# greysun/GraphEmbeddings

Hardware: AMD Instinct MI355X
Metric: scored triples/sec/GPU (d=200) (higher is better)
Workload: dtype f32

## Files before the change

### graphembeddings_amd/csrc/ge_launch.h

```cpp
#pragma once
#include <assert.h>
#include <hip/hip_runtime.h>
#include <stddef.h>
#include <stdint.h>

#include "ge_step_id.h"
#include "ge_sweep_route.h"
#include "ge_trans.h"

namespace ge {

struct TileGeom;
struct ShardOut;

int complex_max_dim();
bool complex_shape_ok(int32_t d, const void* table);
int complex_score_launch(const float* table, int64_t N, int32_t d, const int32_t* triples, int64_t B, float max_norm,
                         int apply_sigmoid, float* out, hipStream_t st, int spectral = 0, float label = 0.f, float l2 = 0.f,
                         const float* table_sumsq = nullptr, int64_t ld = 0);
int complex_hinge_loss_launch(const float* table, int64_t N, int32_t d, const int32_t* pos, const int32_t* neg, int64_t B,
                              float margin, float max_norm, float* loss, float* sig_out, hipStream_t st, int spectral = 0);
int complex_hinge_grad_launch(const float* rows, int64_t N, int32_t d, const int32_t* pos, const int32_t* neg, int64_t B,
                              float margin, float lr, float max_norm, float* loss, int32_t* grad_idx, float* grad_val,
                              hipStream_t st, hipEvent_t ev_start = nullptr, hipEvent_t ev_stop = nullptr,
                              const int32_t* slot_item = nullptr, float* table_rw = nullptr, int spectral = 0,
                              const int32_t* order = nullptr);
int complex_logloss_grad_launch(const float* rows, int64_t N, int32_t d, const int32_t* triples, const float* labels,
                                int64_t M, float lr, float max_norm, float l2, const float* table_sumsq, float* loss,
                                int32_t* grad_idx, float* grad_val, hipStream_t st, const int32_t* negs = nullptr,
                                int64_t B = 0, float row_scale = 1.f, float neg_lr_eff = 0.f, hipEvent_t ev_start = nullptr,
                                hipEvent_t ev_stop = nullptr);
int shard_hinge_grad_launch(float* shard, int32_t d, const float* staged, const int32_t* pos_src, const int32_t* neg_src,
                            const int32_t* slot_item, int32_t R, int64_t B, float margin, float lr, float max_norm,
                            float* loss, int32_t* grad_idx, float* grad_val, float* gsum, int spectral, hipStream_t st,
                            hipEvent_t ev_start, hipEvent_t ev_stop, const int32_t* order, const float* const* peers,
                            int n_peers);
int table_sumsq_launch(const float* table, int64_t n, float* out, hipStream_t st);
int table_scale_launch(float* table, int64_t n, float factor, hipStream_t st);

int hole_max_dim();
int hole_score_launch(const float* table, int64_t N, int32_t d, const int32_t* triples, int64_t B, float max_norm,
                      int apply_sigmoid, float* out, hipStream_t st);
int hole_hinge_loss_launch(const float* table, int64_t N, int32_t d, const int32_t* pos, const int32_t* neg, int64_t B,
                           float margin, float max_norm, float* loss, float* sig_out, hipStream_t st);
int hole_hinge_grad_launch(const float* rows, int64_t N, int32_t d, const int32_t* pos, const int32_t* neg, int64_t B,
                           float margin, float lr, float max_norm, float* loss, int32_t* grad_idx, float* grad_val,
                           hipStream_t st, hipEvent_t ev_start = nullptr, hipEvent_t ev_stop = nullptr);

int hole_spectral_launch(float* table, int64_t N, int32_t d, int inverse, hipStream_t st);

int scatter_add_rows_launch(float* table, int64_t N, int32_t d, const int32_t* idx, const float* val, int64_t R,
                            hipStream_t st, hipEvent_t ev_start = nullptr, hipEvent_t ev_stop = nullptr);
int gather_rows_launch(const float* table, int64_t N, int32_t d, const int32_t* idx, int64_t R, float* out, hipStream_t st);
int corrupt_batch_launch(const int32_t* pos, int64_t B, const TypeSampler& ts, uint64_t step, int32_t* neg, hipStream_t st);
struct SamplerArgs {
  const int32_t* triples; int64_t T; const int64_t* bh_key; const int32_t* bh_ent; const int64_t* bt_key;
  const int32_t* bt_ent; int64_t n_known; const uint32_t* tail_threshold; int32_t n_rel, n_ent;
};
int bernoulli_corrupt_launch(const int32_t* pos, int64_t B, const SamplerArgs& s, int32_t ent_lo, uint64_t seed,
                             uint64_t step, int32_t* neg, hipStream_t st);
int select_rows_launch(const int32_t* valid, int64_t V, int64_t B, uint64_t seed, uint64_t counter, int32_t* out,
                       hipStream_t st);
int mean_pocket_launch(const float* loss, int64_t B, float* mean_out, float* best, int32_t* flag, hipStream_t st);
int copy_if_launch(const float* src, float* dst, int64_t n, const int32_t* flag, hipStream_t st);
bool copy_if_ok(const float* src, const float* dst, int64_t n);
constexpr int kCopyIfChunk = 8192;
// ... 6 lines not shown
int rank_metrics_launch(const int32_t* n_before, const int32_t* n_known_before, const float* true_loss, int64_t M,
                        float* metrics_out, float* best, int32_t* improved, hipStream_t st);

int complex_score_1vK_launch(const float* table, int64_t N, int32_t d, const int32_t* hr, int64_t B, const int32_t* cand,
                             int64_t K, float max_norm, int apply_sigmoid, int cand_is_head, float* out, hipStream_t st);

struct SweepArgs {
  const float* table; int64_t N; int32_t d; const int32_t* hr; int64_t B; const int32_t* true_id; const int32_t* cand;
  int64_t K; float max_norm; int cand_is_head; const int32_t* known_off; const uint16_t* known_rc; int32_t* raw_cnt;
  int32_t* skip_cnt; float* true_loss; float* scores_out; int spec, scores_only, sweep_flags;
};
inline int table_mod16(const SweepArgs& a) { return (int)(reinterpret_cast<uintptr_t>(a.table) % 16); }
struct TopkOut { int32_t k; int32_t* out_id; float* out_loss; void* workspace; size_t workspace_bytes; };
struct SetArgs {
  const int32_t* row_set; const uint32_t* mask; int32_t n_sets;
  int64_t mw;
};

int complex_rank_1vK_launch(const SweepArgs& a, const void* planes_ws, hipStream_t st);

int pipe_sweep_launch(int cw, const SweepArgs& a, hipStream_t st);

int rank_planes_launch(const float* table, int64_t N, int32_t d, const int32_t* cand, int64_t K, float max_norm, int spec,
                       void* planes_ws, hipStream_t st);
int f16_sweep_launch(const SweepArgs& a, const void* planes_ws, hipStream_t st);
int topk_f16_launch(const SweepArgs& a, const TopkOut& t, const void* planes_ws, hipStream_t st);

int64_t candidate_mask_words(int64_t K);
int mask_from_classes_launch(const int32_t* cand_class, int64_t K, const uint32_t* allow, int32_t n_sets, int32_t n_class,
                             uint32_t* mask, hipStream_t st);
int mask_from_cells_launch(const int32_t* cells, int64_t M, int32_t n_sets, int64_t K, uint32_t* mask, hipStream_t st);
int masked_rank_launch(const SweepArgs& a, const SetArgs& sets, const void* planes_ws, hipStream_t st);
int masked_topk_launch(const SweepArgs& a, const TopkOut& t, const SetArgs& sets, const void* planes_ws, hipStream_t st);

int neighbor_max_k();
int neighbor_max_dim();
int64_t neighbor_planes_bytes(int64_t K, int32_t d);
int neighbor_planes_launch(const float* table, int64_t N, int32_t d, const int32_t* cand, int64_t K, void* planes_ws,
                           hipStream_t st);
size_t neighbor_ws_bytes(int64_t B, int64_t K, int32_t k);
int neighbor_dists_launch(const float* table, int64_t N, int32_t d, const int32_t* queries, int64_t B,
                          const int32_t* cand, int64_t K, int metric, const void* planes_ws, float* out, hipStream_t st);
int neighbor_topk_launch(const float* table, int64_t N, int32_t d, const int32_t* queries, int64_t B,
                         const int32_t* cand, int64_t K, int32_t k, int metric, int exclude_self, const void* planes_ws,
                         int32_t* out_id, float* out_dist, void* workspace, size_t workspace_bytes, hipStream_t st);

int known_cells_launch(int pass, const int64_t* key, const int64_t* ent, int64_t M, const int64_t* fixed, const int64_t* rel,
                       int64_t B, const int64_t* pos_of, int64_t n_rows, int64_t n_cand, int32_t* tile_cnt, int32_t* off,
                       uint16_t* rc, hipStream_t st);

size_t sort_scratch_bytes(int64_t n, int64_t n_sub, int64_t P);
unsigned long long* sort_scratch_keys(void* scratch);
int sort_tiles_launch(void* scratch, int64_t n, int64_t n_sub, int64_t P, int64_t n_rows, hipStream_t st,
                      const unsigned* limit, const unsigned long long** sorted);
int items_launch(const unsigned long long* sorted, int64_t n, const TileGeom& G, int direct, int32_t* out, const ShardOut* so,
                 hipStream_t st);
int relation_order_launch(const int32_t* triples, int64_t T, int64_t first_row, int64_t B, int64_t s0, int64_t n, int64_t N,
                          int32_t* out, int64_t stride, int64_t off_order, void* scratch, hipStream_t st);
size_t prep_big_scratch_bytes(int64_t B, int64_t negs, int64_t n);
int prepare_big_launch(const StepSeq& q, int64_t s0, int64_t n, const TypeSampler& ts, int direct, int32_t* out,
                       void* scratch, hipStream_t st, int negs);

int apply_items_launch(float* table, int d, const TileGeom& G, const int32_t* step_rec, const int32_t* gidx,
                       const float* gval, int split, float* out2, hipStream_t st, hipEvent_t ev_start, hipEvent_t ev_stop,
                       int det);
template <class T>
inline T* ws_at(void* base, size_t off) { return reinterpret_cast<T*>(reinterpret_cast<uintptr_t>(base) + off); }
struct HingeWs { int32_t* gidx; float* gval; size_t bytes; };
HingeWs hinge_ws(void* base, int64_t B, int32_t d);
struct LoglossWs { float* sumsq; int32_t* gidx; float* gval; size_t bytes; };
LoglossWs logloss_ws(void* base, int64_t M, int32_t d);
struct StepHyper {
  float lr0, decay_steps, decay_rate, max_norm;
  float lr_at(uint64_t gs) const { return decay_steps > 0.f ? lr0 / (1.0f + decay_rate * ((float)gs / decay_steps)) : lr0; }
};
size_t train_ws_bytes(int64_t B, int32_t d);
int train_steps_run(float* table, int32_t d, const StepSeq& q, int64_t n_steps, const TypeSampler& ts, float margin,
                    const StepHyper& hp, int model, float* loss, int keep_all_losses, int32_t* neg_ws, void* workspace,
                    size_t workspace_bytes, void** ev_pairs, int ev_kernel, void* pipe_handle, hipStream_t st);
size_t train_logloss_ws_bytes(int64_t B, int32_t negs, int32_t d);
int train_logloss_run(float* table, int32_t d, const StepSeq& q, int64_t n_steps, const TypeSampler& ts, int32_t negs,
                      float l2, const StepHyper& hp, float* loss, int keep_all_losses, int32_t* neg_ws, void* workspace,
                      size_t workspace_bytes, void* pipe_handle, hipStream_t st);
size_t train_prepare_bytes(int64_t B, int64_t n_steps);
int train_prepare_run(const StepSeq& q, int64_t n_steps, const TypeSampler& ts, int direct, int32_t* out, hipStream_t st);
void train_prepared_layout(int64_t B, int64_t* out);
int64_t train_chunk_steps(int64_t B, int64_t negs);
int train_adagrad_run(float* table, float* accum, int32_t d, const StepSeq& q, int64_t n_steps, const TypeSampler& ts,
                      float margin, const StepHyper& hp, int model, float* loss, int keep_all_losses, int32_t* neg_ws,
                      void* workspace, size_t workspace_bytes, void* pipe_handle, hipStream_t st);
int pipeline_create(void** out);
int pipeline_reset(void* h);
int pipeline_destroy(void* h);

int adagrad_items_launch(float* table, float* accum, int d, const TileGeom& G, const int32_t* step_rec, const int32_t* gidx,
                         float* gval, float lr, hipStream_t st);
int adagrad_rows_launch(float* table, float* accum, int64_t N, int32_t d, const int32_t* idx, const float* val,
                        const int32_t* perm, int64_t R, float lr, hipStream_t st);

struct SoftmaxWs { float* qp; float* cp; int32_t* qkey; int32_t* ckey; float* lse; float4* part; float* gq; size_t bytes; };
SoftmaxWs softmax_ws(void* base, int64_t B, int64_t K, int32_t d);
size_t softmax_ws_bytes(int64_t B, int64_t K, int32_t d);
int softmax_launch(const float* table, int64_t N, int32_t d, const int32_t* hr, int64_t B, const int32_t* true_id,
                   const int32_t* cand, int64_t K, float max_norm, float scale, float lr, int cand_is_head, float* loss,
                   int32_t* grad_idx, float* grad_val, void* workspace, hipStream_t st);
int softmax_prepare_launch(const float* table, int64_t N, int32_t d, const int32_t* hr, int64_t B, const int32_t* true_id,
                           const int32_t* cand, int64_t K, float max_norm, int cand_is_head, const int32_t* row_set,
                           int32_t n_sets, const SoftmaxWs& w, hipStream_t st);
// ... 174 lines not shown
```

### graphembeddings_amd/csrc/ge_prep.h

```cpp
#pragma once
#include "ge_common.h"

namespace ge {

constexpr int kSlotDirect = -2;
constexpr int kPrepThreads = 1024;
constexpr int kPrepWaves = kPrepThreads / kWave;
constexpr int kItemCap = 16;
constexpr int64_t kSub = 4096;
constexpr int kMaxRadix = 256;
constexpr unsigned long long kInvalidKey = ~0ull;

__host__ __device__ inline int64_t step_row(int64_t first_row, int64_t T, int64_t B, int64_t s) {
  int64_t first = first_row % T;
  if (first + B > T) first = 0;
  const int64_t n0 = (T - first) / B;
  if (s < n0) return first + s * B;
  const int64_t per = T / B;
  return ((s - n0) % per) * B;
}

struct PrepLayout {
  int64_t B, negs, units, n_sub, S, P, off_slot, off_order, off_sub, sub_stride, off_items, off_islots, stride;
  int epu;
// ... 5 lines not shown
  L.epu = negs > 0 ? 3 : 4;
  L.units = negs > 0 ? (1 + negs) * B : B;
  L.n_sub = (L.units + kSub - 1) / kSub;
  const int64_t s = L.units < kSub ? L.units : kSub;
  const int64_t gran = negs > 0 ? 1024 : 256;
  L.S = (s + gran - 1) / gran * gran;
  L.P = L.epu * L.S;
  L.off_slot = 3 * B;
  L.off_order = (negs == 0 && L.n_sub > 1) ? 9 * B : -1;
  L.off_sub = negs > 0 ? (3 * negs * B + 63) / 64 * 64 : ((L.off_order >= 0 ? 10 : 9) * B + 63) / 64 * 64;
  L.off_items = 64;
  L.off_islots = 64 + 2 * L.P;
  L.sub_stride = 64 + 2 * L.P + kItemCap * L.P;
  L.stride = L.off_sub + L.n_sub * L.sub_stride;
  return L;
}

struct TileGeom {
  int P, n_sub;
  int64_t stride;
  int64_t off_slot;
  int64_t off_sub, sub_stride;
  int off_items, off_islots;
};
inline TileGeom geom_of(const PrepLayout& L) {
  return TileGeom{(int)L.P, (int)L.n_sub, L.stride, L.off_slot, L.off_sub, L.sub_stride, (int)L.off_items, (int)L.off_islots};
}
inline TileGeom geom_plain(int P, int n_sub) {
  const int64_t sub = 64 + 2 * (int64_t)P + kItemCap * (int64_t)P;
  return TileGeom{P, n_sub, n_sub * sub, -1, 0, sub, 64, 64 + 2 * P};
}

struct ShardOut {
  int32_t R;
  int64_t B;
  int32_t* pos_src;
  int32_t* neg_src;
  int32_t* req_row;
  const int32_t* tile_heads;
  int32_t peer;
};

struct SortBits { int n_pass, bits; };
inline SortBits sort_bits_for(int64_t N) {
  int nbits = 1;
  while (((int64_t)1 << nbits) <= N) ++nbits;
  SortBits s;
  s.n_pass = (nbits + 7) / 8;
  s.bits = (nbits + s.n_pass - 1) / s.n_pass;
  if (s.bits < 6) s.bits = 6;
  return s;
}

__device__ __forceinline__ int wave_incl_add(int v, int lane) {
#pragma unroll
  for (int o = 1; o < kWave; o <<= 1) { const int t = __shfl_up(v, o, kWave); if (lane >= o) v += t; }
  return v;
}
__device__ __forceinline__ int wave_incl_max(int v, int lane) {
#pragma unroll
  for (int o = 1; o < kWave; o <<= 1) { const int t = __shfl_up(v, o, kWave); if (lane >= o) v = max(v, t); }
  return v;
}

struct StepSource {
  const int32_t* pos; int64_t B; const int32_t* id_to_type; int64_t N; const int64_t* type_offsets;
  int32_t n_types; const int32_t* type_ids; uint64_t seed, step; int32_t padded_size, mode, negs;
};

__device__ __forceinline__ void unit_keys(const StepSource& S, int64_t j, bool batch_heads, int32_t* __restrict__ neg,
                                          unsigned long long (&k)[4]) {
  if (S.negs > 0) {
    const int64_t B = S.B;
    const int64_t i = j < B ? j : (j - B) % B;
    int32_t t3[3] = {S.pos[3 * i], S.pos[3 * i + 1], S.pos[3 * i + 2]};
    if (j >= B) {
      const int64_t kk = (j - B) / B;
      const uint64_t stepk = S.step * (uint64_t)S.negs + (uint64_t)kk;
      const bool heads_k = (S.mode == GE_CORRUPT_BATCH_COIN) ? batch_coin_heads(S.seed, stepk) : false;
      int col;
      const int32_t repl = corrupt_one(t3, i, heads_k, S.id_to_type, S.N, S.type_offsets, S.n_types, S.type_ids, S.seed,
                                       stepk, S.padded_size, S.mode, col);
      t3[col] = repl;
      int32_t* o = neg + 3 * (kk * B + i);
      o[0] = t3[0]; o[1] = t3[1]; o[2] = t3[2];
    }
    const bool bad = t3[0] < 0 || t3[1] < 0 || t3[2] < 0 || t3[0] >= S.N || t3[1] >= S.N || t3[2] >= S.N;
#pragma unroll
    for (int X = 0; X < 3; ++X)
      k[X] = bad ? kInvalidKey : (((unsigned long long)(uint32_t)t3[X] << 32) | (uint32_t)(3 * j + X));
    k[3] = kInvalidKey;
    return;
  }
  const int64_t i = j;
  int32_t p[3] = {S.pos[3 * i], S.pos[3 * i + 1], S.pos[3 * i + 2]};
  int col;
  const int32_t repl = corrupt_one(p, i, batch_heads, S.id_to_type, S.N, S.type_offsets, S.n_types, S.type_ids, S.seed,
                                   S.step, S.padded_size, S.mode, col);
  int32_t n[3] = {p[0], p[1], p[2]};
  n[col] = repl;
  neg[3 * i] = n[0]; neg[3 * i + 1] = n[1]; neg[3 * i + 2] = n[2];
  const bool bad = p[0] < 0 || p[1] < 0 || p[2] < 0 || p[0] >= S.N || p[1] >= S.N || p[2] >= S.N || repl < 0 || repl >= S.N;
#pragma unroll
  for (int X = 0; X < 3; ++X)
    k[X] = bad ? kInvalidKey : (((unsigned long long)(uint32_t)p[X] << 32) | (uint32_t)(6 * i + X));
  k[3] = (bad || repl == p[col]) ? kInvalidKey : (((unsigned long long)(uint32_t)repl << 32) | (uint32_t)(6 * i + 3 + col));
// ... 4 lines not shown
```

### graphembeddings_amd/csrc/ge_prep_big.hip

```cpp
#include "ge_prep.h"
#include "ge_launch.h"
#include <algorithm>

namespace ge {

__global__ __launch_bounds__(kPrepThreads) void prep_big_keys_kernel(
    const int32_t* __restrict__ triples, int64_t T, int64_t first_row, int64_t B, int64_t s0,
    const int32_t* __restrict__ id_to_type, int64_t N, const int64_t* __restrict__ type_offsets,
    int32_t n_types, const int32_t* __restrict__ type_ids, uint64_t seed, uint64_t global_step0,
    int32_t padded_size, int32_t mode, int direct, int negs, int32_t* __restrict__ prep,
    unsigned long long* __restrict__ keys_out) {
  const PrepLayout L = prep_layout(B, negs);
  const int tid = threadIdx.x, sub = blockIdx.y;
  const int64_t s = s0 + blockIdx.x;
  int32_t* rec = prep + (int64_t)blockIdx.x * L.stride;
  int32_t* slot_item = rec + L.off_slot;
  const int64_t i0 = (int64_t)sub * kSub;
  const int S = (int)((L.units - i0) < kSub ? (L.units - i0) : kSub);
  StepSource src{triples + 3 * step_row(first_row, T, B, s), B, id_to_type, N, type_offsets, n_types, type_ids, seed,
                 global_step0 + (uint64_t)s, padded_size, mode, negs};
  const bool batch_heads = (mode == GE_CORRUPT_BATCH_COIN) ? batch_coin_heads(seed, src.step) : false;
  unsigned long long* out = keys_out + ((int64_t)blockIdx.x * L.n_sub + sub) * L.P;
  if (direct)
    for (int i = tid; i < 6 * S; i += kPrepThreads) slot_item[6 * i0 + i] = -1;
  for (int il = tid; il < (int)L.S; il += kPrepThreads) {
    unsigned long long k[4] = {kInvalidKey, kInvalidKey, kInvalidKey, kInvalidKey};
    if (il < S) unit_keys(src, i0 + il, batch_heads, rec, k);
#pragma unroll
    for (int X = 0; X < 4; ++X)
      if (X < L.epu) out[L.epu * il + X] = k[X];
  }
}

__device__ __forceinline__ bool pass_is_identity(const unsigned* limit, int shift) {
  return limit && ((unsigned long long)(*limit) >> (shift - 32)) == 0ull;
}

__global__ __launch_bounds__(kPrepThreads) void prep_big_hist_kernel(
    const unsigned long long* __restrict__ src, int P, int n_sub, int shift, int bits, unsigned* __restrict__ hist,
    const unsigned* __restrict__ limit) {
  __shared__ unsigned cnt[kMaxRadix];
  if (pass_is_identity(limit, shift)) return;
  const int tid = threadIdx.x, tile = blockIdx.y;
  const int radix = 1 << bits;
  const unsigned dmask = (unsigned)radix - 1u;
  if (tid < radix) cnt[tid] = 0;
  __syncthreads();
  const unsigned long long* k = src + ((int64_t)blockIdx.x * n_sub + tile) * P;
  for (int i = tid; i < P; i += kPrepThreads) atomicAdd(&cnt[(unsigned)(k[i] >> shift) & dmask], 1u);
  __syncthreads();
  if (tid < radix) hist[((int64_t)blockIdx.x * radix + tid) * n_sub + tile] = cnt[tid];
}

__global__ __launch_bounds__(kPrepThreads) void prep_big_scatter_kernel(
    const unsigned long long* __restrict__ src, unsigned long long* __restrict__ dst,
    const unsigned* __restrict__ hist, int P, int n_sub, int shift, int bits, const unsigned* __restrict__ limit) {
  __shared__ unsigned whist[kMaxRadix * kPrepWaves];
  __shared__ unsigned gbase[kMaxRadix];
  __shared__ unsigned dstart[kMaxRadix];
  __shared__ unsigned wsum[4], wsum2[4];
  extern __shared__ __attribute__((aligned(16))) unsigned long long lkeys[];
  const int tid = threadIdx.x, lane = tid & (kWave - 1), wave = tid >> 6, tile = blockIdx.y;
  if (pass_is_identity(limit, shift)) {
    const int64_t o = ((int64_t)blockIdx.x * n_sub + tile) * P;
    for (int i = tid; i < P; i += kPrepThreads) dst[o + i] = src[o + i];
    return;
  }
  const int radix = 1 << bits, R = P / kPrepThreads, seg = kWave * R;
  const unsigned dmask = (unsigned)radix - 1u;
  const unsigned* h = hist + (int64_t)blockIdx.x * radix * n_sub;
  unsigned tot = 0, before = 0, mine = 0;
  if (tid < radix)
    for (int q = 0; q < n_sub; ++q) { const unsigned v = h[tid * n_sub + q]; if (q < tile) before += v; if (q == tile) mine = v; tot += v; }
  int incl = 0, incl2 = 0;
  if (tid < kMaxRadix) {
    incl = wave_incl_add((int)tot, lane);
    incl2 = wave_incl_add((int)mine, lane);
    if (lane == kWave - 1) { wsum[wave] = (unsigned)incl; wsum2[wave] = (unsigned)incl2; }
  }
  for (int i = tid; i < radix * kPrepWaves; i += kPrepThreads) whist[i] = 0;
  __syncthreads();
  if (tid < radix) {
    unsigned run = (unsigned)incl - tot, run2 = (unsigned)incl2 - mine;
    for (int w = 0; w < wave; ++w) { run += wsum[w]; run2 += wsum2[w]; }
    gbase[tid] = run + before;
    dstart[tid] = run2;
  }
  const unsigned long long* kin = src + ((int64_t)blockIdx.x * n_sub + tile) * P;
  unsigned long long k[16];
  unsigned off[16];
#pragma unroll
  for (int r = 0; r < 16; ++r)
    if (r < R) k[r] = kin[wave * seg + r * kWave + lane];
#pragma unroll
  for (int r = 0; r < 16; ++r) {
    if (r < R) {
      const unsigned dg = (unsigned)(k[r] >> shift) & dmask;
      unsigned long long peers = ~0ull;
      for (int b = 0; b < bits; ++b) {
        const bool bit = (dg >> b) & 1u;
        const unsigned long long bal = __ballot(bit);
        peers &= bit ? bal : ~bal;
      }
      const unsigned rank = (unsigned)__popcll(peers & ((1ull << lane) - 1ull));
      const unsigned cnt = (unsigned)__popcll(peers);
      unsigned* hp = whist + dg * kPrepWaves + wave;
      const unsigned base = *hp;
      __builtin_amdgcn_wave_barrier();
      if (rank == 0) *hp = base + cnt;
      __builtin_amdgcn_wave_barrier();
      off[r] = base + rank;
    }
  }
  __syncthreads();
  if (tid < radix) {
    unsigned run = 0;
    for (int w = 0; w < kPrepWaves; ++w) { const unsigned c = whist[tid * kPrepWaves + w]; whist[tid * kPrepWaves + w] = run; run += c; }
  }
  __syncthreads();
#pragma unroll
  for (int r = 0; r < 16; ++r) {
    if (r < R) {
      const unsigned dg = (unsigned)(k[r] >> shift) & dmask;
      lkeys[dstart[dg] + whist[dg * kPrepWaves + wave] + off[r]] = k[r];
    }
  }
  __syncthreads();
  unsigned long long* out = dst + (int64_t)blockIdx.x * n_sub * P;
  for (int i = tid; i < P; i += kPrepThreads) {
    const unsigned long long kk = lkeys[i];
    const unsigned dg = (unsigned)(kk >> shift) & dmask;
    out[gbase[dg] + ((unsigned)i - dstart[dg])] = kk;
  }
}

template <bool SHARD>
__global__ __launch_bounds__(kPrepThreads) void prep_big_items_kernel(
    const unsigned long long* __restrict__ sorted, TileGeom G, int direct, int32_t* __restrict__ prep, ShardOut so) {
  extern __shared__ __attribute__((aligned(16))) unsigned long long keys[];
  const int P = G.P, R = P / kPrepThreads, seg = kWave * R, n_sub = G.n_sub;
  int* wtot = reinterpret_cast<int*>(keys + P);
  const int tid = threadIdx.x, lane = tid & (kWave - 1), wave = tid >> 6, tile = blockIdx.y;
  const unsigned long long* g = sorted + (int64_t)blockIdx.x * n_sub * P;
  const int total = n_sub * P, base = tile * P;
  int32_t* rec = prep + (int64_t)blockIdx.x * G.stride;
  int32_t* slot_item = G.off_slot >= 0 ? rec + G.off_slot : nullptr;
  int32_t* subrec = rec + G.off_sub + tile * G.sub_stride;
  int32_t* items = subrec + G.off_items;
  int32_t* islots = subrec + G.off_islots;
  for (int i = tid; i < P; i += kPrepThreads) keys[i] = g[base + i];
  if (tid == 0) {
    int rs = -1;
    if (tile > 0) {
      const unsigned long long k0 = g[base], kp = g[base - 1];
      const uint32_t r0 = (uint32_t)(k0 >> 32);
      if (k0 != kInvalidKey && (uint32_t)(kp >> 32) == r0) {
        int lo = 0, hi = base - 1;
        while (lo < hi) { const int mid = (lo + hi) >> 1; if ((uint32_t)(g[mid] >> 32) < r0) lo = mid + 1; else hi = mid; }
        rs = lo;
      }
    }
    wtot[31] = rs;
    int before = 0;
    if (SHARD)
      for (int t = 0; t < tile; ++t) before += so.tile_heads[(int64_t)blockIdx.x * n_sub + t];
    wtot[30] = before;
  }
  __syncthreads();
  const int rs_in = wtot[31], u_before = wtot[30];
  auto key_at = [&](int i) -> unsigned long long {
    if (i >= 0 && i < P) return keys[i];
    const int gi = base + i;
    return (gi >= 0 && gi < total) ? g[gi] : kInvalidKey;
  };
  {
    int carry = -1;
    for (int r = 0; r < R; ++r) {
      const int i = wave * seg + r * kWave + lane;
      const unsigned long long kk = keys[i], kp = key_at(i - 1);
      const bool head = kk != kInvalidKey && (base + i == 0 || (uint32_t)(kp >> 32) != (uint32_t)(kk >> 32));
      const int m = max(wave_incl_max(head ? base + i : -1, lane), carry);
      carry = __shfl(m, kWave - 1, kWave);
    }
    if (lane == 0) wtot[wave] = carry;
  }
  __syncthreads();
  int prev_max = rs_in;
  for (int w = 0; w < wave; ++w) prev_max = max(prev_max, wtot[w]);
  __syncthreads();
  unsigned start_mask = 0, sole_mask = 0, rhead_mask = 0;
  int inc_loc[16], rs_loc[16];
  {
    int carry = 0, mcarry = prev_max;
#pragma unroll
    for (int r = 0; r < 16; ++r) {
      if (r < R) {
        const int i = wave * seg + r * kWave + lane;
        const unsigned long long kk = keys[i], kp = key_at(i - 1), kn = key_at(i + 1);
        const bool valid = kk != kInvalidKey;
        const uint32_t row = (uint32_t)(kk >> 32);
        const bool head = valid && (base + i == 0 || (uint32_t)(kp >> 32) != row);
        const bool sole = direct && head && !(kn != kInvalidKey && (uint32_t)(kn >> 32) == row) &&
                          !(SHARD && so.peer && row < (uint32_t)so.R);
        const bool rhead = SHARD && head && row >= (uint32_t)so.R;
        const int rs = max(wave_incl_max(head ? base + i : -1, lane), mcarry);
        mcarry = __shfl(rs, kWave - 1, kWave);
        rs_loc[r] = rs;
        const bool start = valid && ((base + i - rs) % kItemCap) == 0 && !sole;
        if (start) start_mask |= 1u << r;
        if (sole) sole_mask |= 1u << r;
        if (rhead) rhead_mask |= 1u << r;
        const int incl = wave_incl_add((start ? 1 : 0) | (rhead ? 1 << 16 : 0), lane) + carry;
        inc_loc[r] = incl;
        carry = __shfl(incl, kWave - 1, kWave);
      }
    }
    if (lane == 0) wtot[wave] = carry;
  }
  __syncthreads();
  int prev = 0, all = 0;
  for (int w = 0; w < kPrepWaves; ++w) { if (w < wave) prev += wtot[w]; all += wtot[w]; }
  if (tid == 0) subrec[0] = all & 0xFFFF;
// ... 14 lines not shown
        uint32_t src = row;
        if (remote) {
          if ((rhead_mask >> r) & 1u) so.req_row[(int64_t)blockIdx.x * total + u] = (int32_t)(row % (uint32_t)so.R);
          if (!so.peer) src = (uint32_t)so.R + (uint32_t)u;
          row = (uint32_t)so.R + (uint32_t)u;
          tag = -3 - u;
        }
        const uint32_t pair = slot / 6u, X = slot - pair * 6u;
        if (X < 3) so.pos_src[((int64_t)blockIdx.x * so.B + pair) * 3 + X] = (int32_t)src;
        else so.neg_src[(int64_t)blockIdx.x * so.B + pair] = (int32_t)((src << 1) | (X - 3u));
      }
      if (sole) slot_item[slot] = tag;
      const bool is_start = (start_mask >> r) & 1u;
      unsigned long long sm = __ballot(is_start);
      const int idx_me = prev_items + (inc_loc[r] & 0xFFFF) - 1;
      const int g16 = lane >> 4, j16 = lane & 15;
      while (sm) {
        int srcl = -1;
#pragma unroll
        for (int g = 0; g < 4; ++g) {
          const int bpos = sm ? __builtin_ctzll(sm) : -1;
          if (sm) sm &= sm - 1;
          if (g == g16) srcl = bpos;
        }
        const int sl = srcl < 0 ? 0 : srcl;
        const int i_s = wave * seg + r * kWave + sl;
        const int idx_s = __shfl(idx_me, sl, kWave);
        const int row_s = __shfl((int)row, sl, kWave);
        const int rs_s = __shfl(rs_loc[r], sl, kWave);
        const unsigned long long k0 = key_at(i_s);
        const uint32_t krow = (uint32_t)(k0 >> 32);
        const unsigned long long kj = key_at(i_s + j16);
        const bool same = srcl >= 0 && kj != kInvalidKey && (uint32_t)(kj >> 32) == krow;
        const unsigned m16 = (unsigned)((__ballot(same) >> (16 * g16)) & 0xFFFFull);
        const int cnt = m16 == 0xFFFFu ? kItemCap : __builtin_ctz(~m16);
        if (srcl >= 0) {
          islots[idx_s * kItemCap + j16] = j16 < cnt ? (int32_t)(uint32_t)kj : -1;
          if (j16 == 0) {
            bool more = false;
            if (cnt == kItemCap) { const unsigned long long ke = key_at(i_s + kItemCap); more = ke != kInvalidKey && (uint32_t)(ke >> 32) == krow; }
            const bool multi = (base + i_s != rs_s) || more;
            items[2 * idx_s] = row_s;
            items[2 * idx_s + 1] = cnt | (multi ? (1 << 30) : 0);
          }
        }
      }
    }
  }
}

constexpr int kOrderP = 16384;
__global__ __launch_bounds__(kPrepThreads) void order_keys_kernel(
    const int32_t* __restrict__ triples, int64_t T, int64_t first_row, int64_t B, int64_t s0, int64_t N, int n_o,
    unsigned long long* __restrict__ keys_out, unsigned* __restrict__ limit) {
  const int64_t s = blockIdx.x;
  unsigned rmax = 0;
  const int32_t* pos = T > 0 ? triples + 3 * step_row(first_row, T, B, s0 + s) : triples + s * 3 * B;
  unsigned long long* out = keys_out + (s * n_o + blockIdx.y) * kOrderP;
  for (int i = threadIdx.x; i < kOrderP; i += kPrepThreads) {
    const int64_t j = (int64_t)blockIdx.y * kOrderP + i;
    unsigned long long k = kInvalidKey;
    if (j < B) {
      int32_t r = pos[3 * j + 2];
      if (r < 0 || r >= N) r = (int32_t)N;
      k = ((unsigned long long)(uint32_t)r << 32) | (uint32_t)j;
      rmax = max(rmax, (unsigned)r);
    }
    out[i] = k;
  }
#pragma unroll
  for (int m = 32; m >= 1; m >>= 1) rmax = max(rmax, (unsigned)__shfl_xor((int)rmax, m, kWave));
  if ((threadIdx.x & (kWave - 1)) == 0) atomicMax(limit, rmax);
}

__global__ __launch_bounds__(kPrepThreads) void order_write_kernel(
    const unsigned long long* __restrict__ sorted, int n_o, int64_t B, int64_t stride, int64_t off_order,
    int32_t* __restrict__ prep) {
  const unsigned long long* g = sorted + (int64_t)blockIdx.x * n_o * kOrderP;
  int32_t* order = prep + (int64_t)blockIdx.x * stride + off_order;
  for (int64_t i = (int64_t)blockIdx.y * kPrepThreads + threadIdx.x; i < B; i += (int64_t)gridDim.y * kPrepThreads)
    order[i] = (int32_t)(uint32_t)g[i];
}

size_t sort_scratch_bytes(int64_t n, int64_t n_sub, int64_t P) {
  const size_t keys = align_up(sizeof(unsigned long long) * (size_t)n * (size_t)n_sub * (size_t)P, 256);
  const size_t hist = align_up(sizeof(unsigned) * (size_t)n * kMaxRadix * (size_t)n_sub, 256);
  return 2 * keys + hist + 256;
}
static unsigned* sort_scratch_limit(void* scratch, int64_t n, int64_t n_sub, int64_t P) {
  return reinterpret_cast<unsigned*>(reinterpret_cast<char*>(scratch) + sort_scratch_bytes(n, n_sub, P) - 256);
}
unsigned long long* sort_scratch_keys(void* scratch) { return reinterpret_cast<unsigned long long*>(scratch); }

int sort_tiles_launch(void* scratch, int64_t n, int64_t n_sub, int64_t P, int64_t n_rows, hipStream_t st,
                      const unsigned* limit, const unsigned long long** sorted) {
  const SortBits sb = sort_bits_for(n_rows);
  const size_t keys_bytes = align_up(sizeof(unsigned long long) * (size_t)n * (size_t)n_sub * (size_t)P, 256);
  unsigned long long* ka = reinterpret_cast<unsigned long long*>(scratch);
  unsigned long long* kb = reinterpret_cast<unsigned long long*>(reinterpret_cast<char*>(scratch) + keys_bytes);
  unsigned* hist = reinterpret_cast<unsigned*>(reinterpret_cast<char*>(scratch) + 2 * keys_bytes);
  const dim3 grid((unsigned)n, (unsigned)n_sub), block(kPrepThreads);
  const size_t lds = sizeof(unsigned long long) * (size_t)P;
  const hipError_t e = hipFuncSetAttribute(reinterpret_cast<const void*>(prep_big_scatter_kernel),
                                           hipFuncAttributeMaxDynamicSharedMemorySize, 140 * 1024);
  if (e != hipSuccess) return (int)e;
  for (int pass = 0; pass < sb.n_pass; ++pass) {
    const int shift = 32 + pass * sb.bits;
    hipLaunchKernelGGL(prep_big_hist_kernel, grid, block, 0, st, ka, (int)P, (int)n_sub, shift, sb.bits, hist, limit);
    hipLaunchKernelGGL(prep_big_scatter_kernel, grid, block, lds, st, ka, kb, hist, (int)P, (int)n_sub, shift, sb.bits, limit);
    unsigned long long* t = ka; ka = kb; kb = t;
  }
  *sorted = ka;
  return launch_status();
}

int items_launch(const unsigned long long* sorted, int64_t n, const TileGeom& G, int direct, int32_t* out, const ShardOut* so,
                 hipStream_t st) {
  const size_t lds = sizeof(unsigned long long) * (size_t)G.P + sizeof(int) * 32;
  const dim3 grid((unsigned)n, (unsigned)G.n_sub), block(kPrepThreads);
  if (so) {
    hipError_t e = hipFuncSetAttribute(reinterpret_cast<const void*>(prep_big_items_kernel<true>),
                                       hipFuncAttributeMaxDynamicSharedMemorySize, 160 * 1024);
    if (e != hipSuccess) return (int)e;
    hipLaunchKernelGGL(prep_big_items_kernel<true>, grid, block, lds, st, sorted, G, direct, out, *so);
  } else {
    hipError_t e = hipFuncSetAttribute(reinterpret_cast<const void*>(prep_big_items_kernel<false>),
                                       hipFuncAttributeMaxDynamicSharedMemorySize, 160 * 1024);
    if (e != hipSuccess) return (int)e;
    hipLaunchKernelGGL(prep_big_items_kernel<false>, grid, block, lds, st, sorted, G, direct, out, ShardOut{});
  }
  return launch_status();
}

int relation_order_launch(const int32_t* triples, int64_t T, int64_t first_row, int64_t B, int64_t s0, int64_t n, int64_t N,
                          int32_t* out, int64_t stride, int64_t off_order, void* scratch, hipStream_t st) {
  const int n_o = (int)((B + kOrderP - 1) / kOrderP);
  unsigned* limit = sort_scratch_limit(scratch, n, n_o, kOrderP);
  if (hipMemsetAsync(limit, 0, sizeof(unsigned), st) != hipSuccess) return launch_status();
  hipLaunchKernelGGL(order_keys_kernel, dim3((unsigned)n, (unsigned)n_o), dim3(kPrepThreads), 0, st, triples, T, first_row, B,
                     s0, N, n_o, sort_scratch_keys(scratch), limit);
  const unsigned long long* sorted;
  const int rc = sort_tiles_launch(scratch, n, n_o, kOrderP, N + 1, st, limit, &sorted);
  if (rc) return rc;
  const int gy = (int)std::min<int64_t>((B + kPrepThreads - 1) / kPrepThreads, 64);
  hipLaunchKernelGGL(order_write_kernel, dim3((unsigned)n, (unsigned)gy), dim3(kPrepThreads), 0, st, sorted, n_o, B, stride,
                     off_order, out);
  return launch_status();
}

size_t prep_big_scratch_bytes(int64_t B, int64_t negs, int64_t n) {
  const PrepLayout L = prep_layout(B, negs);
  return L.n_sub <= 1 ? 0 : sort_scratch_bytes(n, L.n_sub, L.P);
}

int prepare_big_launch(const StepSeq& q, int64_t s0, int64_t n, const TypeSampler& ts, int direct, int32_t* out,
                       void* scratch, hipStream_t st, int negs) {
  const PrepLayout L = prep_layout(q.B, negs);
  const dim3 grid((unsigned)n, (unsigned)L.n_sub), block(kPrepThreads);
  hipLaunchKernelGGL(prep_big_keys_kernel, grid, block, 0, st, q.triples, q.T, q.first_row, q.B, s0, ts.id_to_type, ts.N,
                     ts.type_offsets, ts.n_types, ts.type_ids, ts.seed, q.global_step0, ts.padded_size, ts.mode, direct, negs,
                     out, sort_scratch_keys(scratch));
  const unsigned long long* sorted;
  int rc = sort_tiles_launch(scratch, n, L.n_sub, L.P, ts.N, st, nullptr, &sorted);
  if (rc) return rc;
  rc = items_launch(sorted, n, geom_of(L), direct, out, nullptr, st);
  if (rc || L.off_order < 0) return rc;
  return relation_order_launch(q.triples, q.T, q.first_row, q.B, s0, n, ts.N, out, L.stride, L.off_order, scratch, st);
}

}
```

### graphembeddings_amd/csrc/ge_shard.hip

```cpp
#include "ge_prep.h"
#include "ge_launch.h"

namespace ge {

__global__ __launch_bounds__(kPrepThreads) void shard_keys_kernel(
    const int32_t* __restrict__ pos, const int32_t* __restrict__ neg, int64_t B, int64_t N, int32_t G, int32_t rank,
    int32_t R, PrepLayout L, int32_t* __restrict__ prep, int32_t* __restrict__ pos_src, int32_t* __restrict__ neg_src,
    unsigned long long* __restrict__ keys_out) {
  const int tid = threadIdx.x, sub = blockIdx.y;
  const int64_t s = blockIdx.x;
  int32_t* slot_item = prep + s * L.stride + L.off_slot;
  const int64_t i0 = (int64_t)sub * kSub;
  const int S = (int)((B - i0) < kSub ? (B - i0) : kSub);
  unsigned long long* out = keys_out + (s * L.n_sub + sub) * L.P;
  for (int i = tid; i < 6 * S; i += kPrepThreads) slot_item[6 * i0 + i] = -1;
  auto vrow = [&](int32_t id) -> unsigned long long {
    const int32_t o = id % G, l = id / G;
    return (unsigned long long)(uint32_t)(o == rank ? l : R * (1 + o) + l);
  };
  for (int il = tid; il < (int)L.S; il += kPrepThreads) {
    unsigned long long k[4] = {kInvalidKey, kInvalidKey, kInvalidKey, kInvalidKey};
    if (il < S) {
      const int64_t i = i0 + il;
      const int32_t* p = pos + (s * B + i) * 3;
// ... 23 lines not shown
  const int tid = threadIdx.x, tile = blockIdx.y;
  const unsigned long long* g = sorted + (int64_t)blockIdx.x * n_sub * P;
  const int base = tile * P;
  if (tid <= 64) own[tid] = 0;
  __syncthreads();
  for (int i = tid; i < P; i += kPrepThreads) {
    const unsigned long long kk = g[base + i];
    if (kk == kInvalidKey) continue;
    const uint32_t row = (uint32_t)(kk >> 32);
    const bool head = (base + i == 0) || (uint32_t)(g[base + i - 1] >> 32) != row;
    if (!head) continue;
    if (row < (uint32_t)R) { atomicAdd(&own[rank], 1); continue; }
    atomicAdd(&own[row / (uint32_t)R - 1], 1);
    atomicAdd(&own[64], 1);
  }
  __syncthreads();
  if (tid < G && own[tid]) atomicAdd(&counts[(int64_t)blockIdx.x * G + tid], own[tid]);
  if (tid == 0) tile_heads[(int64_t)blockIdx.x * n_sub + tile] = own[64];
}

__global__ __launch_bounds__(kPrepThreads) void owner_keys_kernel(
    const int32_t* __restrict__ req_all, const int64_t* __restrict__ req_start, int P, int n_sub, int32_t rows_local,
    unsigned long long* __restrict__ keys_out) {
  const int64_t s = blockIdx.x;
  const int64_t b = req_start[s], n = req_start[s + 1] - b;
  unsigned long long* out = keys_out + (s * n_sub + blockIdx.y) * P;
  for (int i = threadIdx.x; i < P; i += kPrepThreads) {
    const int64_t j = (int64_t)blockIdx.y * P + i;
    unsigned long long k = kInvalidKey;
    if (j < n) {
      const int32_t row = req_all[b + j];
      if (row >= 0 && row < rows_local) k = ((unsigned long long)(uint32_t)row << 32) | (uint32_t)j;
    }
    out[i] = k;
  }
}

size_t shard_plan_scratch_bytes(int64_t B, int64_t S) {
  const PrepLayout L = prep_layout(B);
  return sort_scratch_bytes(S, L.n_sub, L.P) + align_up(sizeof(int32_t) * (size_t)S * (size_t)L.n_sub, 256);
}

int shard_plan_launch(const int32_t* pos, const int32_t* neg, int64_t S, int64_t B, int64_t N, int32_t G, int32_t rank,
                      int32_t* records, int32_t* pos_src, int32_t* neg_src, int32_t* req_row, int32_t* counts,
                      void* scratch, int peer, hipStream_t st) {
  const PrepLayout L = prep_layout(B);
  const int32_t R = (int32_t)((N + G - 1) / G);
  const dim3 grid((unsigned)S, (unsigned)L.n_sub), block(kPrepThreads);
  int32_t* tile_heads = reinterpret_cast<int32_t*>(reinterpret_cast<char*>(scratch) + sort_scratch_bytes(S, L.n_sub, L.P));
  hipError_t e = hipMemsetAsync(counts, 0, sizeof(int32_t) * (size_t)S * (size_t)G, st);
  if (e != hipSuccess) return (int)e;
  hipLaunchKernelGGL(shard_keys_kernel, grid, block, 0, st, pos, neg, B, N, G, rank, R, L, records, pos_src, neg_src,
                     sort_scratch_keys(scratch));
  const unsigned long long* sorted;
  int rc = sort_tiles_launch(scratch, S, L.n_sub, L.P, (int64_t)R * (G + 1), st, nullptr, &sorted);
  if (rc) return rc;
  hipLaunchKernelGGL(shard_heads_kernel, grid, block, 0, st, sorted, (int)L.P, (int)L.n_sub, R, G, rank, tile_heads, counts);
  const ShardOut so{R, B, pos_src, neg_src, req_row, tile_heads, peer ? 1 : 0};
  rc = items_launch(sorted, S, geom_of(L), 1, records, &so, st);
  if (rc || L.off_order < 0) return rc;
  return relation_order_launch(pos, 0, 0, B, 0, S, N, records, L.stride, L.off_order, scratch, st);
}

int shard_grad_launch(float* shard, int32_t d, const float* staged, const int32_t* pos_src, const int32_t* neg_src,
                      const int32_t* record, int32_t R, int64_t B, float margin, float lr, float max_norm, int spectral,
                      float* loss, int32_t* gidx, float* gval, float* gsum, const float* const* peers, int n_peers,
                      hipStream_t st, hipEvent_t e0, hipEvent_t e1) {
  const PrepLayout L = prep_layout(B);
  return shard_hinge_grad_launch(shard, d, staged, pos_src, neg_src, record + L.off_slot, R, B, margin, lr, max_norm, loss,
                                 gidx, gval, gsum, spectral, st, e0, e1, L.off_order >= 0 ? record + L.off_order : nullptr,
                                 peers, n_peers);
}

int shard_apply_launch(float* shard, int32_t d, const int32_t* record, int64_t B, const int32_t* gidx, const float* gval,
                       int32_t R, float* gsum, hipStream_t st, hipEvent_t e0, hipEvent_t e1) {
  return apply_items_launch(shard, d, geom_of(prep_layout(B)), record, gidx, gval, R, gsum, st, e0, e1, 0);
}

constexpr int kOwnerP = 16384;
static inline int owner_tiles(int64_t cap) { return (int)((cap + kOwnerP - 1) / kOwnerP); }
int64_t shard_owner_record_words(int64_t cap) { return cap <= 0 ? 0 : geom_plain(kOwnerP, owner_tiles(cap)).stride; }
size_t shard_owner_scratch_bytes(int64_t cap, int64_t S) { return cap <= 0 ? 0 : sort_scratch_bytes(S, owner_tiles(cap), kOwnerP); }

int shard_owner_plan_launch(const int32_t* req_all, const int64_t* req_start, int64_t S, int64_t cap, int32_t rows_local,
                            int32_t* records, void* scratch, hipStream_t st) {
  if (cap <= 0 || S <= 0) return 0;
  const int n_sub = owner_tiles(cap);
  const dim3 grid((unsigned)S, (unsigned)n_sub), block(kPrepThreads);
  hipLaunchKernelGGL(owner_keys_kernel, grid, block, 0, st, req_all, req_start, kOwnerP, n_sub, rows_local,
                     sort_scratch_keys(scratch));
  const unsigned long long* sorted;
  const int rc = sort_tiles_launch(scratch, S, n_sub, kOwnerP, rows_local, st, nullptr, &sorted);
  if (rc) return rc;
  return items_launch(sorted, S, geom_plain(kOwnerP, n_sub), 0, records, nullptr, st);
}

int shard_owner_apply_launch(float* shard, int32_t d, const int32_t* record, int64_t cap, const float* recv, hipStream_t st) {
  if (cap <= 0) return 0;
  return apply_items_launch(shard, d, geom_plain(kOwnerP, owner_tiles(cap)), record, nullptr, recv, 0x7FFFFFFF, nullptr, st,
                            nullptr, nullptr, 0);
}

}
```

Baseline: 628.3 million.

## Fuse first radix histogram into key kernels and skip identity-pass copies

The key-generation kernels now build the first radix-pass digit histogram in shared memory using wave-ballot aggregated atomics, so the first histogram kernel launch is skipped. Identity scatter passes no longer copy keys; instead a SortedKeys descriptor picks the correct ping-pong buffer on the device from the limit value. The boundary binary search in the items kernel becomes a block-parallel search, and the histogram kernel also uses ballot-aggregated counting. This removes a launch and key-buffer read/copy traffic from preprocessing, at the cost of extra ballot work per key and more complex buffer selection logic.

```diff
diff --git a/graphembeddings_amd/csrc/ge_launch.h b/graphembeddings_amd/csrc/ge_launch.h
--- a/graphembeddings_amd/csrc/ge_launch.h
+++ b/graphembeddings_amd/csrc/ge_launch.h
@@ -12,6 +12,7 @@
 
 struct TileGeom;
 struct ShardOut;
+struct SortedKeys;
 
 int complex_max_dim();
 bool complex_shape_ok(int32_t d, const void* table);
@@ -124,8 +125,8 @@
 size_t sort_scratch_bytes(int64_t n, int64_t n_sub, int64_t P);
 unsigned long long* sort_scratch_keys(void* scratch);
 int sort_tiles_launch(void* scratch, int64_t n, int64_t n_sub, int64_t P, int64_t n_rows, hipStream_t st,
-                      const unsigned* limit, const unsigned long long** sorted);
-int items_launch(const unsigned long long* sorted, int64_t n, const TileGeom& G, int direct, int32_t* out, const ShardOut* so,
+                      const unsigned* limit, bool counted0, SortedKeys* sorted);
+int items_launch(const SortedKeys& sorted, int64_t n, const TileGeom& G, int direct, int32_t* out, const ShardOut* so,
                  hipStream_t st);
 int relation_order_launch(const int32_t* triples, int64_t T, int64_t first_row, int64_t B, int64_t s0, int64_t n, int64_t N,
                           int32_t* out, int64_t stride, int64_t off_order, void* scratch, hipStream_t st);
diff --git a/graphembeddings_amd/csrc/ge_prep.h b/graphembeddings_amd/csrc/ge_prep.h
--- a/graphembeddings_amd/csrc/ge_prep.h
+++ b/graphembeddings_amd/csrc/ge_prep.h
@@ -81,6 +81,29 @@
   return s;
 }
 
+struct SortedKeys {
+  const unsigned long long *a, *b;
+  const unsigned* limit;
+  int bits, n_pass;
+  __device__ __forceinline__ const unsigned long long* get() const {
+    if (!limit) return a;
+    const unsigned long long lim = *limit;
+    int real = 0;
+    for (int p = 0; p < n_pass; ++p) real += (lim >> (p * bits)) != 0ull;
+    return (real & 1) ? b : a;
+  }
+};
+
+__device__ __forceinline__ void count_digit(unsigned* cnt, unsigned idx, int nbits, int lane) {
+  unsigned long long peers = __ballot(1);
+  for (int b = 0; b < nbits; ++b) {
+    const bool bit = (idx >> b) & 1u;
+    const unsigned long long bal = __ballot(bit);
+    peers &= bit ? bal : ~bal;
+  }
+  if ((peers & ((1ull << lane) - 1ull)) == 0ull) atomicAdd(&cnt[idx], (unsigned)__popcll(peers));
+}
+
 __device__ __forceinline__ int wave_incl_add(int v, int lane) {
 #pragma unroll
   for (int o = 1; o < kWave; o <<= 1) { const int t = __shfl_up(v, o, kWave); if (lane >= o) v += t; }
diff --git a/graphembeddings_amd/csrc/ge_prep_big.hip b/graphembeddings_amd/csrc/ge_prep_big.hip
--- a/graphembeddings_amd/csrc/ge_prep_big.hip
+++ b/graphembeddings_amd/csrc/ge_prep_big.hip
@@ -3,15 +3,26 @@
 #include <algorithm>
 
 namespace ge {
+
+struct PassCounts { unsigned* hist; int bits; };
+
+__device__ __forceinline__ void publish_counts(const unsigned* cnt, const PassCounts& pc, int64_t step, int n_sub, int tile) {
+  const int radix = 1 << pc.bits;
+  for (int i = threadIdx.x; i < radix; i += kPrepThreads) pc.hist[(step * radix + i) * n_sub + tile] = cnt[i];
+}
 
 __global__ __launch_bounds__(kPrepThreads) void prep_big_keys_kernel(
     const int32_t* __restrict__ triples, int64_t T, int64_t first_row, int64_t B, int64_t s0,
     const int32_t* __restrict__ id_to_type, int64_t N, const int64_t* __restrict__ type_offsets,
     int32_t n_types, const int32_t* __restrict__ type_ids, uint64_t seed, uint64_t global_step0,
     int32_t padded_size, int32_t mode, int direct, int negs, int32_t* __restrict__ prep,
-    unsigned long long* __restrict__ keys_out) {
+    unsigned long long* __restrict__ keys_out, PassCounts pc) {
+  __shared__ unsigned cnt[kMaxRadix];
   const PrepLayout L = prep_layout(B, negs);
   const int tid = threadIdx.x, sub = blockIdx.y;
+  const unsigned dmask = (1u << pc.bits) - 1u;
+  if (tid < kMaxRadix) cnt[tid] = 0;
+  __syncthreads();
   const int64_t s = s0 + blockIdx.x;
   int32_t* rec = prep + (int64_t)blockIdx.x * L.stride;
   int32_t* slot_item = rec + L.off_slot;
@@ -28,8 +39,13 @@
     if (il < S) unit_keys(src, i0 + il, batch_heads, rec, k);
 #pragma unroll
     for (int X = 0; X < 4; ++X)
-      if (X < L.epu) out[L.epu * il + X] = k[X];
-  }
+      if (X < L.epu) {
+        out[L.epu * il + X] = k[X];
+        count_digit(cnt, (unsigned)(k[X] >> 32) & dmask, pc.bits, tid & (kWave - 1));
+      }
+  }
+  __syncthreads();
+  publish_counts(cnt, pc, blockIdx.x, (int)L.n_sub, sub);
 }
 
 __device__ __forceinline__ bool pass_is_identity(const unsigned* limit, int shift) {
@@ -47,9 +63,9 @@
   if (tid < radix) cnt[tid] = 0;
   __syncthreads();
   const unsigned long long* k = src + ((int64_t)blockIdx.x * n_sub + tile) * P;
-  for (int i = tid; i < P; i += kPrepThreads) atomicAdd(&cnt[(unsigned)(k[i] >> shift) & dmask], 1u);
-  __syncthreads();
-  if (tid < radix) hist[((int64_t)blockIdx.x * radix + tid) * n_sub + tile] = cnt[tid];
+  for (int i = tid; i < P; i += kPrepThreads) count_digit(cnt, (unsigned)(k[i] >> shift) & dmask, bits, tid & (kWave - 1));
+  __syncthreads();
+  publish_counts(cnt, PassCounts{hist, bits}, blockIdx.x, n_sub, tile);
 }
 
 __global__ __launch_bounds__(kPrepThreads) void prep_big_scatter_kernel(
@@ -61,11 +77,7 @@
   __shared__ unsigned wsum[4], wsum2[4];
   extern __shared__ __attribute__((aligned(16))) unsigned long long lkeys[];
   const int tid = threadIdx.x, lane = tid & (kWave - 1), wave = tid >> 6, tile = blockIdx.y;
-  if (pass_is_identity(limit, shift)) {
-    const int64_t o = ((int64_t)blockIdx.x * n_sub + tile) * P;
-    for (int i = tid; i < P; i += kPrepThreads) dst[o + i] = src[o + i];
-    return;
-  }
+  if (pass_is_identity(limit, shift)) return;
   const int radix = 1 << bits, R = P / kPrepThreads, seg = kWave * R;
   const unsigned dmask = (unsigned)radix - 1u;
   const unsigned* h = hist + (int64_t)blockIdx.x * radix * n_sub;
@@ -136,12 +148,12 @@
 
 template <bool SHARD>
 __global__ __launch_bounds__(kPrepThreads) void prep_big_items_kernel(
-    const unsigned long long* __restrict__ sorted, TileGeom G, int direct, int32_t* __restrict__ prep, ShardOut so) {
+    SortedKeys sorted, TileGeom G, int direct, int32_t* __restrict__ prep, ShardOut so) {
   extern __shared__ __attribute__((aligned(16))) unsigned long long keys[];
   const int P = G.P, R = P / kPrepThreads, seg = kWave * R, n_sub = G.n_sub;
   int* wtot = reinterpret_cast<int*>(keys + P);
   const int tid = threadIdx.x, lane = tid & (kWave - 1), wave = tid >> 6, tile = blockIdx.y;
-  const unsigned long long* g = sorted + (int64_t)blockIdx.x * n_sub * P;
+  const unsigned long long* g = sorted.get() + (int64_t)blockIdx.x * n_sub * P;
   const int total = n_sub * P, base = tile * P;
   int32_t* rec = prep + (int64_t)blockIdx.x * G.stride;
   int32_t* slot_item = G.off_slot >= 0 ? rec + G.off_slot : nullptr;
@@ -149,25 +161,38 @@
   int32_t* items = subrec + G.off_items;
   int32_t* islots = subrec + G.off_islots;
   for (int i = tid; i < P; i += kPrepThreads) keys[i] = g[base + i];
+  int rs_in = -1;
+  if (tile > 0) {
+    const unsigned long long k0 = g[base], kp = g[base - 1];
+    const uint32_t r0 = (uint32_t)(k0 >> 32);
+    if (k0 != kInvalidKey && (uint32_t)(kp >> 32) == r0) {
+      int lo = 0, hi = base - 1;
+      while (lo < hi) {
+        const int step = (hi - lo + kPrepThreads - 1) / kPrepThreads;
+        const int pos = lo + tid * step;
+        const bool before = pos < hi && (uint32_t)(g[pos] >> 32) < r0;
+        if (tid == 0) wtot[29] = 0;
+        __syncthreads();
+        const unsigned long long bal = __ballot(before);
+        if (lane == 0 && bal) atomicAdd(&wtot[29], (int)__popcll(bal));
+        __syncthreads();
+        const int F = wtot[29];
+        __syncthreads();
+        const int nhi = min(lo + F * step, hi);
+        lo = F ? lo + (F - 1) * step + 1 : lo;
+        hi = F ? nhi : lo;
+      }
+      rs_in = lo;
+    }
+  }
   if (tid == 0) {
-    int rs = -1;
-    if (tile > 0) {
-      const unsigned long long k0 = g[base], kp = g[base - 1];
-      const uint32_t r0 = (uint32_t)(k0 >> 32);
-      if (k0 != kInvalidKey && (uint32_t)(kp >> 32) == r0) {
-        int lo = 0, hi = base - 1;
-        while (lo < hi) { const int mid = (lo + hi) >> 1; if ((uint32_t)(g[mid] >> 32) < r0) lo = mid + 1; else hi = mid; }
-        rs = lo;
-      }
-    }
-    wtot[31] = rs;
     int before = 0;
     if (SHARD)
       for (int t = 0; t < tile; ++t) before += so.tile_heads[(int64_t)blockIdx.x * n_sub + t];
     wtot[30] = before;
   }
   __syncthreads();
-  const int rs_in = wtot[31], u_before = wtot[30];
+  const int u_before = wtot[30];
   auto key_at = [&](int i) -> unsigned long long {
     if (i >= 0 && i < P) return keys[i];
     const int gi = base + i;
@@ -288,8 +313,12 @@
 constexpr int kOrderP = 16384;
 __global__ __launch_bounds__(kPrepThreads) void order_keys_kernel(
     const int32_t* __restrict__ triples, int64_t T, int64_t first_row, int64_t B, int64_t s0, int64_t N, int n_o,
-    unsigned long long* __restrict__ keys_out, unsigned* __restrict__ limit) {
+    unsigned long long* __restrict__ keys_out, unsigned* __restrict__ limit, PassCounts pc) {
+  __shared__ unsigned cnt[kMaxRadix];
   const int64_t s = blockIdx.x;
+  const unsigned dmask = (1u << pc.bits) - 1u;
+  if (threadIdx.x < kMaxRadix) cnt[threadIdx.x] = 0;
+  __syncthreads();
   unsigned rmax = 0;
   const int32_t* pos = T > 0 ? triples + 3 * step_row(first_row, T, B, s0 + s) : triples + s * 3 * B;
   unsigned long long* out = keys_out + (s * n_o + blockIdx.y) * kOrderP;
@@ -303,54 +332,63 @@
       rmax = max(rmax, (unsigned)r);
     }
     out[i] = k;
-  }
+    count_digit(cnt, (unsigned)(k >> 32) & dmask, pc.bits, threadIdx.x & (kWave - 1));
+  }
+  __syncthreads();
+  publish_counts(cnt, pc, s, n_o, blockIdx.y);
 #pragma unroll
   for (int m = 32; m >= 1; m >>= 1) rmax = max(rmax, (unsigned)__shfl_xor((int)rmax, m, kWave));
   if ((threadIdx.x & (kWave - 1)) == 0) atomicMax(limit, rmax);
 }
 
 __global__ __launch_bounds__(kPrepThreads) void order_write_kernel(
-    const unsigned long long* __restrict__ sorted, int n_o, int64_t B, int64_t stride, int64_t off_order,
-    int32_t* __restrict__ prep) {
-  const unsigned long long* g = sorted + (int64_t)blockIdx.x * n_o * kOrderP;
+    SortedKeys sorted, int n_o, int64_t B, int64_t stride, int64_t off_order, int32_t* __restrict__ prep) {
+  const unsigned long long* g = sorted.get() + (int64_t)blockIdx.x * n_o * kOrderP;
   int32_t* order = prep + (int64_t)blockIdx.x * stride + off_order;
   for (int64_t i = (int64_t)blockIdx.y * kPrepThreads + threadIdx.x; i < B; i += (int64_t)gridDim.y * kPrepThreads)
     order[i] = (int32_t)(uint32_t)g[i];
 }
 
+static size_t sort_keys_bytes(int64_t n, int64_t n_sub, int64_t P) {
+  return align_up(sizeof(unsigned long long) * (size_t)n * (size_t)n_sub * (size_t)P, 256);
+}
 size_t sort_scratch_bytes(int64_t n, int64_t n_sub, int64_t P) {
-  const size_t keys = align_up(sizeof(unsigned long long) * (size_t)n * (size_t)n_sub * (size_t)P, 256);
   const size_t hist = align_up(sizeof(unsigned) * (size_t)n * kMaxRadix * (size_t)n_sub, 256);
-  return 2 * keys + hist + 256;
+  return 2 * sort_keys_bytes(n, n_sub, P) + hist + 256;
 }
 static unsigned* sort_scratch_limit(void* scratch, int64_t n, int64_t n_sub, int64_t P) {
   return reinterpret_cast<unsigned*>(reinterpret_cast<char*>(scratch) + sort_scratch_bytes(n, n_sub, P) - 256);
 }
 unsigned long long* sort_scratch_keys(void* scratch) { return reinterpret_cast<unsigned long long*>(scratch); }
+static PassCounts sort_pass_counts(void* scratch, int64_t n, int64_t n_sub, int64_t P, int64_t n_rows) {
+  return PassCounts{reinterpret_cast<unsigned*>(reinterpret_cast<char*>(scratch) + 2 * sort_keys_bytes(n, n_sub, P)),
+                    sort_bits_for(n_rows).bits};
+}
 
 int sort_tiles_launch(void* scratch, int64_t n, int64_t n_sub, int64_t P, int64_t n_rows, hipStream_t st,
-                      const unsigned* limit, const unsigned long long** sorted) {
+                      const unsigned* limit, bool counted0, SortedKeys* sorted) {
   const SortBits sb = sort_bits_for(n_rows);
-  const size_t keys_bytes = align_up(sizeof(unsigned long long) * (size_t)n * (size_t)n_sub * (size_t)P, 256);
+  unsigned* hist = sort_pass_counts(scratch, n, n_sub, P, n_rows).hist;
   unsigned long long* ka = reinterpret_cast<unsigned long long*>(scratch);
-  unsigned long long* kb = reinterpret_cast<unsigned long long*>(reinterpret_cast<char*>(scratch) + keys_bytes);
-  unsigned* hist = reinterpret_cast<unsigned*>(reinterpret_cast<char*>(scratch) + 2 * keys_bytes);
+  unsigned long long* kb = reinterpret_cast<unsigned long long*>(reinterpret_cast<char*>(scratch) + sort_keys_bytes(n, n_sub, P));
   const dim3 grid((unsigned)n, (unsigned)n_sub), block(kPrepThreads);
   const size_t lds = sizeof(unsigned long long) * (size_t)P;
   const hipError_t e = hipFuncSetAttribute(reinterpret_cast<const void*>(prep_big_scatter_kernel),
                                            hipFuncAttributeMaxDynamicSharedMemorySize, 140 * 1024);
   if (e != hipSuccess) return (int)e;
+  *sorted = limit ? SortedKeys{ka, kb, limit, sb.bits, sb.n_pass}
+                  : SortedKeys{(sb.n_pass & 1) ? kb : ka, (sb.n_pass & 1) ? ka : kb, nullptr, sb.bits, sb.n_pass};
   for (int pass = 0; pass < sb.n_pass; ++pass) {
     const int shift = 32 + pass * sb.bits;
-    hipLaunchKernelGGL(prep_big_hist_kernel, grid, block, 0, st, ka, (int)P, (int)n_sub, shift, sb.bits, hist, limit);
+    if (pass > 0 || !counted0)
+      hipLaunchKernelGGL(prep_big_hist_kernel, grid, block, 0, st, ka, (int)P, (int)n_sub, shift, sb.bits, hist, limit);
     hipLaunchKernelGGL(prep_big_scatter_kernel, grid, block, lds, st, ka, kb, hist, (int)P, (int)n_sub, shift, sb.bits, limit);
     unsigned long long* t = ka; ka = kb; kb = t;
   }
-  *sorted = ka;
   return launch_status();
 }
 
-int items_launch(const unsigned long long* sorted, int64_t n, const TileGeom& G, int direct, int32_t* out, const ShardOut* so,
+int items_launch(const SortedKeys& sorted, int64_t n, const TileGeom& G, int direct, int32_t* out, const ShardOut* so,
                  hipStream_t st) {
   const size_t lds = sizeof(unsigned long long) * (size_t)G.P + sizeof(int) * 32;
   const dim3 grid((unsigned)n, (unsigned)G.n_sub), block(kPrepThreads);
@@ -374,9 +412,9 @@
   unsigned* limit = sort_scratch_limit(scratch, n, n_o, kOrderP);
   if (hipMemsetAsync(limit, 0, sizeof(unsigned), st) != hipSuccess) return launch_status();
   hipLaunchKernelGGL(order_keys_kernel, dim3((unsigned)n, (unsigned)n_o), dim3(kPrepThreads), 0, st, triples, T, first_row, B,
-                     s0, N, n_o, sort_scratch_keys(scratch), limit);
-  const unsigned long long* sorted;
-  const int rc = sort_tiles_launch(scratch, n, n_o, kOrderP, N + 1, st, limit, &sorted);
+                     s0, N, n_o, sort_scratch_keys(scratch), limit, sort_pass_counts(scratch, n, n_o, kOrderP, N + 1));
+  SortedKeys sorted;
+  const int rc = sort_tiles_launch(scratch, n, n_o, kOrderP, N + 1, st, limit, true, &sorted);
   if (rc) return rc;
   const int gy = (int)std::min<int64_t>((B + kPrepThreads - 1) / kPrepThreads, 64);
   hipLaunchKernelGGL(order_write_kernel, dim3((unsigned)n, (unsigned)gy), dim3(kPrepThreads), 0, st, sorted, n_o, B, stride,
@@ -395,9 +433,9 @@
   const dim3 grid((unsigned)n, (unsigned)L.n_sub), block(kPrepThreads);
   hipLaunchKernelGGL(prep_big_keys_kernel, grid, block, 0, st, q.triples, q.T, q.first_row, q.B, s0, ts.id_to_type, ts.N,
                      ts.type_offsets, ts.n_types, ts.type_ids, ts.seed, q.global_step0, ts.padded_size, ts.mode, direct, negs,
-                     out, sort_scratch_keys(scratch));
-  const unsigned long long* sorted;
-  int rc = sort_tiles_launch(scratch, n, L.n_sub, L.P, ts.N, st, nullptr, &sorted);
+                     out, sort_scratch_keys(scratch), sort_pass_counts(scratch, n, L.n_sub, L.P, ts.N));
+  SortedKeys sorted;
+  int rc = sort_tiles_launch(scratch, n, L.n_sub, L.P, ts.N, st, nullptr, true, &sorted);
   if (rc) return rc;
   rc = items_launch(sorted, n, geom_of(L), direct, out, nullptr, st);
   if (rc || L.off_order < 0) return rc;
diff --git a/graphembeddings_amd/csrc/ge_shard.hip b/graphembeddings_amd/csrc/ge_shard.hip
--- a/graphembeddings_amd/csrc/ge_shard.hip
+++ b/graphembeddings_amd/csrc/ge_shard.hip
@@ -99,10 +99,10 @@
   if (e != hipSuccess) return (int)e;
   hipLaunchKernelGGL(shard_keys_kernel, grid, block, 0, st, pos, neg, B, N, G, rank, R, L, records, pos_src, neg_src,
                      sort_scratch_keys(scratch));
-  const unsigned long long* sorted;
-  int rc = sort_tiles_launch(scratch, S, L.n_sub, L.P, (int64_t)R * (G + 1), st, nullptr, &sorted);
+  SortedKeys sorted;
+  int rc = sort_tiles_launch(scratch, S, L.n_sub, L.P, (int64_t)R * (G + 1), st, nullptr, false, &sorted);
   if (rc) return rc;
-  hipLaunchKernelGGL(shard_heads_kernel, grid, block, 0, st, sorted, (int)L.P, (int)L.n_sub, R, G, rank, tile_heads, counts);
+  hipLaunchKernelGGL(shard_heads_kernel, grid, block, 0, st, sorted.a, (int)L.P, (int)L.n_sub, R, G, rank, tile_heads, counts);
   const ShardOut so{R, B, pos_src, neg_src, req_row, tile_heads, peer ? 1 : 0};
   rc = items_launch(sorted, S, geom_of(L), 1, records, &so, st);
   if (rc || L.off_order < 0) return rc;
@@ -136,8 +136,8 @@
   const dim3 grid((unsigned)S, (unsigned)n_sub), block(kPrepThreads);
   hipLaunchKernelGGL(owner_keys_kernel, grid, block, 0, st, req_all, req_start, kOwnerP, n_sub, rows_local,
                      sort_scratch_keys(scratch));
-  const unsigned long long* sorted;
-  const int rc = sort_tiles_launch(scratch, S, n_sub, kOwnerP, rows_local, st, nullptr, &sorted);
+  SortedKeys sorted;
+  const int rc = sort_tiles_launch(scratch, S, n_sub, kOwnerP, rows_local, st, nullptr, false, &sorted);
   if (rc) return rc;
   return items_launch(sorted, S, geom_plain(kOwnerP, n_sub), 0, records, nullptr, st);
 }
```

Result: no change. 627.7 million (-0.1%).
